# reazon-research/ReazonSpeech

Measured on NVIDIA H100. Metric: RTFx (audio-s/wall-s) FastConformer-RNNT 619M, higher is better.
Workload: dtype bf16

## Files before the change

reazonspeech_b200/csrc/attention_tc.cu:

```cuda
#include <cuda.h>

#include "common.cuh"
#include "kernels.h"

namespace rs {

namespace {

constexpr int TQ = 128;
constexpr int TDK = 128;
constexpr int KB = 64;
constexpr int kBlocks = 6;
constexpr int kSlab = TQ * 128;
constexpr int kAtcThreads = 32 * 9;
constexpr int kKvStages = 3;
constexpr uint32_t kKvStageBytes = 2 * KB * 128 + TDK * 128;
constexpr uint32_t kOffQ = 0;
constexpr uint32_t kOffKV = 2 * kSlab;
constexpr uint32_t kOffBD = kOffKV + kKvStages * kKvStageBytes;
constexpr int kBdPitch = 296;
constexpr int kNrelPadMax = 288;
constexpr uint32_t kOffBar = kOffBD + TQ * kBdPitch * 2;
constexpr uint32_t kAtcSmem = kOffBar + 1536 + 1024;
constexpr int kOutPitch = 136;
static_assert(2 * kNrelPadMax * 128 <= kKvStages * kKvStageBytes && kOutPitch <= kBdPitch && kAtcSmem <= 227 * 1024, "shared memory layout");

struct AtcDev {
  const __nv_bfloat16* qk;
  const __nv_bfloat16* vt;
  const float* bd_bias;
  const float* bias_u;
  __nv_bfloat16* out;
  const int32_t* enc_len;
  int T_max, H, w_left, w_right, n_global, n_rel_pad, ld_qk, ld_vt;
};

__device__ __forceinline__ float ex2f(float x) { float y; asm("ex2.approx.ftz.f32 %0, %1;" : "=f"(y) : "f"(x)); return y; }

__device__ __forceinline__ uint32_t sw128(int row, int chunk) {
  return static_cast<uint32_t>((row >> 3) * 1024 + (row & 7) * 128 + ((chunk ^ (row & 7)) << 4));
}

__global__ void __launch_bounds__(kAtcThreads, 1)
local_attention_tc_kernel(const __grid_constant__ CUtensorMap tm_q, const __grid_constant__ CUtensorMap tm_k,
                          const __grid_constant__ CUtensorMap tm_vt, const __grid_constant__ CUtensorMap tm_pos, const AtcDev p) {
  extern __shared__ uint8_t atc_raw[];
  const uint32_t base = (smem_u32(atc_raw) + 1023u) & ~1023u;
  uint8_t* gen = atc_raw + (base - smem_u32(atc_raw));
  const uint32_t bar_qk = base + kOffBar, bar_drained = bar_qk + 8;
  auto full_bar = [&](int s) { return bar_qk + 16u + 8u * s; };
  auto empty_bar = [&](int s) { return bar_qk + 40u + 8u * s; };
  __nv_bfloat16* s_k0 = reinterpret_cast<__nv_bfloat16*>(gen + kOffBar + 64);
  float* s_uk = reinterpret_cast<float*>(gen + kOffBar + 320);
  float* s_sg = reinterpret_cast<float*>(gen + kOffBar + 512);
  float* s_v0 = reinterpret_cast<float*>(gen + kOffBar + 1024);

  const int b = blockIdx.z, h = blockIdx.y, q0 = blockIdx.x * TQ;
  const int len = p.enc_len[b];
  const int d = p.H * TDK;
  const int warp = warp_id_uniform(), lane = lane_id();
  const size_t row0 = static_cast<size_t>(b) * p.T_max;
  __nv_bfloat16* obase = p.out + row0 * d + h * TDK;

  if (q0 >= len) {
    for (int id = threadIdx.x; id < TQ * 16; id += blockDim.x) {
      const int r = id >> 4, c = (id & 15) * 8;
      if (q0 + r < p.T_max) *reinterpret_cast<uint4*>(obase + static_cast<size_t>(q0 + r) * d + c) = make_uint4(0, 0, 0, 0);
    }
    return;
  }

  const int j_base = q0 - 128;
  const int q_hi = min(q0 + TQ, len) - 1;
  const int key_lo = max(0, q0 - p.w_left), key_hi = min(len - 1, q_hi + p.w_right);
  const int blk_lo = max((key_lo - j_base) >> 6, 0), blk_hi = min((key_hi - j_base) >> 6, kBlocks - 1);
  const uint32_t pos_slab = static_cast<uint32_t>(p.n_rel_pad) * 128u;

  if (threadIdx.x == 256) {
    tma_prefetch_desc(&tm_q);
    tma_prefetch_desc(&tm_k);
    tma_prefetch_desc(&tm_vt);
    tma_prefetch_desc(&tm_pos);
    mbar_init(bar_qk, 1); mbar_init(bar_drained, 8);
    for (int s = 0; s < kKvStages; ++s) { mbar_init(full_bar(s), 1); mbar_init(empty_bar(s), 8); }
    fence_barrier_init();
    mbar_arrive_expect_tx(bar_qk, static_cast<uint32_t>(2 * kSlab + 2 * pos_slab));
    for (int kb = 0; kb < 2; ++kb) {
      tma_load_2d(base + kOffQ + kb * kSlab, &tm_q, h * TDK + kb * 64, static_cast<int>(row0) + q0, bar_qk);
      for (int hh = 0; hh < 2; ++hh)
        tma_load_2d(base + kOffKV + kb * pos_slab + hh * (pos_slab / 2), &tm_pos, kb * 64, h * p.n_rel_pad + hh * (p.n_rel_pad / 2), bar_qk);
    }
  }
  __syncthreads();

  if (warp == 8) {
    if (lane == 0) {
      mbar_wait(bar_drained, 0);
      int s = 0; uint32_t phase = 0;
      for (int blk = blk_lo; blk <= blk_hi; ++blk) {
        mbar_wait(empty_bar(s), phase ^ 1u);
        mbar_arrive_expect_tx(full_bar(s), kKvStageBytes);
        const uint32_t st = base + kOffKV + s * kKvStageBytes;
        const int key0 = static_cast<int>(row0) + j_base + blk * KB;
        for (int kb = 0; kb < 2; ++kb) tma_load_2d(st + kb * (KB * 128), &tm_k, d + h * TDK + kb * 64, key0, full_bar(s));
        tma_load_2d(st + 2 * KB * 128, &tm_vt, key0, h * TDK, full_bar(s));
        if (++s == kKvStages) { s = 0; phase ^= 1u; }
      }
    }
    return;
  }

  const int wg = warp >> 2, g = lane >> 2, t = lane & 3;
  const int rbase = wg * 64 + (warp & 3) * 16;
  const int r0 = rbase + g, r1 = r0 + 8;
  const int i0 = q0 + r0, i1 = q0 + r1;
  const bool ok0 = i0 < len, ok1 = i1 < len;
  const float scale2 = rsqrtf(static_cast<float>(TDK)) * 1.4426950408889634f;
  __half* s_bd = reinterpret_cast<__half*>(gen + kOffBD);

  float sg0 = -INFINITY, sg1 = -INFINITY;
  if (p.n_global > 0) {
    const int tid = threadIdx.x;
    if (tid < 16) *reinterpret_cast<uint4*>(s_k0 + tid * 8) = __ldg(reinterpret_cast<const uint4*>(p.qk + row0 * p.ld_qk + d + h * TDK) + tid);
    if (tid >= 128) s_v0[tid - 128] = __bfloat162float(p.vt[static_cast<size_t>(h * TDK + (tid - 128)) * p.ld_vt + row0]);
    named_bar_sync(1, 256);
    if (warp == 0) {
      float uk = 0.f;
#pragma unroll
      for (int e = 0; e < 4; ++e) uk = fmaf(__ldg(p.bias_u + h * TDK + lane * 4 + e), __bfloat162float(s_k0[lane * 4 + e]), uk);
      uk = warp_sum(uk);
      if (lane == 0) *s_uk = uk;
    }
    mbar_wait(bar_qk, 0);
    {
      const int r = tid >> 1, hf = tid & 1;
      float acc0 = 0.f, acc1 = 0.f;
#pragma unroll
      for (int c = 0; c < 8; ++c) {
        const uint4 qv = *reinterpret_cast<const uint4*>(gen + kOffQ + hf * kSlab + sw128(r, c));
        const uint4 kv = *reinterpret_cast<const uint4*>(s_k0 + hf * 64 + c * 8);
        const uint32_t qw[4] = {qv.x, qv.y, qv.z, qv.w}, kw[4] = {kv.x, kv.y, kv.z, kv.w};
#pragma unroll
        for (int e = 0; e < 4; ++e) {
          const float2 q2 = unpack_bf16x2(qw[e]), k2 = unpack_bf16x2(kw[e]);
          acc0 = fmaf(q2.x, k2.x, acc0); acc1 = fmaf(q2.y, k2.y, acc1);
        }
      }
      float acc = acc0 + acc1;
      acc += __shfl_xor_sync(0xffffffffu, acc, 1);
      if (hf == 0) s_sg[r] = acc;
    }
    named_bar_sync(1, 256);
    sg0 = (s_sg[r0] - *s_uk) * scale2;
    sg1 = (s_sg[r1] - *s_uk) * scale2;
  } else {
    mbar_wait(bar_qk, 0);
  }

  const uint32_t q_addr = base + kOffQ + wg * (64 * 128);
#pragma unroll 1
  for (int ch = 0; ch < (p.n_rel_pad >> 5); ++ch) {
    float acc[16];
    wgmma_fence();
#pragma unroll
    for (int kb = 0; kb < 2; ++kb) {
      const uint64_t da = wgmma_desc_k_sw128(q_addr + kb * kSlab);
      const uint64_t db = wgmma_desc_k_sw128(base + kOffKV + kb * pos_slab + ch * 4096);
#pragma unroll
      for (int k = 0; k < 4; ++k) wgmma_bf16_ss_n32(acc, da + 2u * k, db + 2u * k, (kb | k) != 0 ? 1u : 0u);
    }
    wgmma_commit();
    wgmma_wait<0>();
#pragma unroll
    for (int j = 0; j < 4; ++j) {
      const int col = ch * 32 + 8 * j + 2 * t;
      const float2 bb = __ldg(reinterpret_cast<const float2*>(p.bd_bias + h * p.n_rel_pad + col));
      *reinterpret_cast<__half2*>(s_bd + r0 * kBdPitch + col) = __floats2half2_rn((acc[4 * j] + bb.x) * scale2, (acc[4 * j + 1] + bb.y) * scale2);
      *reinterpret_cast<__half2*>(s_bd + r1 * kBdPitch + col) = __floats2half2_rn((acc[4 * j + 2] + bb.x) * scale2, (acc[4 * j + 3] + bb.y) * scale2);
    }
  }
  __syncwarp();
  if (lane == 0) mbar_arrive(bar_drained);

  const int wrow_lo = q0 + wg * 64;
  const bool wg_valid = wrow_lo < len;
  const int wkey_lo = max(0, wrow_lo - p.w_left), wkey_hi = min(len - 1, min(wrow_lo + 64, len) - 1 + p.w_right);

  float o[64];
#pragma unroll
  for (int e = 0; e < 64; ++e) o[e] = 0.f;
  float m0 = -INFINITY, m1 = -INFINITY, l0 = 0.f, l1 = 0.f;
  const __half* bd0 = s_bd + r0 * kBdPitch + p.w_left - i0;
  const __half* bd1 = s_bd + r1 * kBdPitch + p.w_left - i1;
  int s = 0; uint32_t phase = 0;
#pragma unroll 1
  for (int blk = blk_lo; blk <= blk_hi; ++blk) {
    mbar_wait(full_bar(s), phase);
    const int jlo = j_base + blk * KB;
    if (wg_valid && jlo + KB - 1 >= wkey_lo && jlo <= wkey_hi) {
      const uint32_t st = base + kOffKV + s * kKvStageBytes;
      float sc[32];
      wgmma_fence();
#pragma unroll
      for (int kb = 0; kb < 2; ++kb) {
        const uint64_t da = wgmma_desc_k_sw128(q_addr + kb * kSlab);
        const uint64_t db = wgmma_desc_k_sw128(st + kb * (KB * 128));
#pragma unroll
        for (int k = 0; k < 4; ++k) wgmma_bf16_ss_n64(sc, da + 2u * k, db + 2u * k, (kb | k) != 0 ? 1u : 0u);
      }
      wgmma_commit();
      wgmma_wait<0>();
      float mx0 = -INFINITY, mx1 = -INFINITY;
#pragma unroll
      for (int j = 0; j < 8; ++j) {
#pragma unroll
        for (int q = 0; q < 2; ++q) {
          const int ja = jlo + 8 * j + 2 * t + q;
          const bool in = ja >= 0 && ja < len;
          const bool a0 = in && ok0 && ja - i0 >= -p.w_left && ja - i0 <= p.w_right;
          const bool a1 = in && ok1 && ja - i1 >= -p.w_left && ja - i1 <= p.w_right;
          const float t0 = a0 ? fmaf(sc[4 * j + q], scale2, __half2float(bd0[ja])) : -INFINITY;
          const float t1 = a1 ? fmaf(sc[4 * j + 2 + q], scale2, __half2float(bd1[ja])) : -INFINITY;
          sc[4 * j + q] = t0; sc[4 * j + 2 + q] = t1;
          mx0 = fmaxf(mx0, t0); mx1 = fmaxf(mx1, t1);
        }
      }
      mx0 = fmaxf(mx0, __shfl_xor_sync(0xffffffffu, mx0, 1)); mx0 = fmaxf(mx0, __shfl_xor_sync(0xffffffffu, mx0, 2));
      mx1 = fmaxf(mx1, __shfl_xor_sync(0xffffffffu, mx1, 1)); mx1 = fmaxf(mx1, __shfl_xor_sync(0xffffffffu, mx1, 2));
      const float n0 = fmaxf(m0, mx0), n1 = fmaxf(m1, mx1);
      const float c0 = m0 == -INFINITY ? 0.f : ex2f(m0 - n0), c1 = m1 == -INFINITY ? 0.f : ex2f(m1 - n1);
      const float ref0 = n0 == -INFINITY ? 0.f : n0, ref1 = n1 == -INFINITY ? 0.f : n1;
      m0 = n0; m1 = n1;
      l0 *= c0; l1 *= c1;
#pragma unroll
      for (int j = 0; j < 16; ++j) { o[4 * j] *= c0; o[4 * j + 1] *= c0; o[4 * j + 2] *= c1; o[4 * j + 3] *= c1; }
      uint32_t pa[4][4];
#pragma unroll
      for (int j = 0; j < 8; ++j) {
        const uint32_t w0 = pack_bf16x2(ex2f(sc[4 * j] - ref0), ex2f(sc[4 * j + 1] - ref0));
        const uint32_t w1 = pack_bf16x2(ex2f(sc[4 * j + 2] - ref1), ex2f(sc[4 * j + 3] - ref1));
        const float2 b0 = unpack_bf16x2(w0), b1 = unpack_bf16x2(w1);
        l0 += b0.x + b0.y; l1 += b1.x + b1.y;
        pa[j >> 1][(j & 1) * 2] = w0; pa[j >> 1][(j & 1) * 2 + 1] = w1;
      }
      wgmma_fence();
      const uint64_t dv = wgmma_desc_k_sw128(st + 2 * KB * 128);
#pragma unroll
      for (int kk = 0; kk < 4; ++kk) wgmma_bf16_rs_n128(o, pa[kk], dv + 2u * kk, 1u);
      wgmma_commit();
      wgmma_wait<0>();
    }
    __syncwarp();
    if (lane == 0) mbar_arrive(empty_bar(s));
    if (++s == kKvStages) { s = 0; phase ^= 1u; }
  }

  l0 += __shfl_xor_sync(0xffffffffu, l0, 1); l0 += __shfl_xor_sync(0xffffffffu, l0, 2);
  l1 += __shfl_xor_sync(0xffffffffu, l1, 1); l1 += __shfl_xor_sync(0xffffffffu, l1, 2);
  float pg0 = 0.f, pg1 = 0.f;
  if (p.n_global > 0) {
    const float f0 = fmaxf(m0, sg0), f1 = fmaxf(m1, sg1);
    const float c0 = m0 == -INFINITY ? 0.f : ex2f(m0 - f0), c1 = m1 == -INFINITY ? 0.f : ex2f(m1 - f1);
    pg0 = ok0 ? ex2f(sg0 - f0) : 0.f; pg1 = ok1 ? ex2f(sg1 - f1) : 0.f;
    l0 = l0 * c0 + pg0; l1 = l1 * c1 + pg1;
#pragma unroll
    for (int j = 0; j < 16; ++j) { o[4 * j] *= c0; o[4 * j + 1] *= c0; o[4 * j + 2] *= c1; o[4 * j + 3] *= c1; }
  }
  const float inv0 = (ok0 && l0 > 0.f) ? 1.0f / l0 : 0.f, inv1 = (ok1 && l1 > 0.f) ? 1.0f / l1 : 0.f;
  __syncwarp();
  __nv_bfloat16* stage = reinterpret_cast<__nv_bfloat16*>(s_bd + rbase * kBdPitch);
#pragma unroll
  for (int j = 0; j < 16; ++j) {
    const int col = 8 * j + 2 * t;
    const float v0a = p.n_global > 0 ? s_v0[col] : 0.f, v0b = p.n_global > 0 ? s_v0[col + 1] : 0.f;
    *reinterpret_cast<uint32_t*>(stage + g * kOutPitch + col) = pack_bf16x2((o[4 * j] + pg0 * v0a) * inv0, (o[4 * j + 1] + pg0 * v0b) * inv0);
    *reinterpret_cast<uint32_t*>(stage + (g + 8) * kOutPitch + col) = pack_bf16x2((o[4 * j + 2] + pg1 * v0a) * inv1, (o[4 * j + 3] + pg1 * v0b) * inv1);
  }
  __syncwarp();
#pragma unroll
  for (int it = 0; it < 8; ++it) {
    const int rr = it * 2 + (lane >> 4), cc = (lane & 15) * 8;
    const int row = q0 + rbase + rr;
    const uint4 a = *reinterpret_cast<const uint4*>(stage + rr * kOutPitch + cc);
    if (row < p.T_max) *reinterpret_cast<uint4*>(obase + static_cast<size_t>(row) * d + cc) = a;
  }
}

__global__ void __launch_bounds__(256)
global_row_attention_tc_kernel(const AtcDev p) {
  extern __shared__ __align__(16) float gs[];
  const int h = blockIdx.x, b = blockIdx.y;
  const int len = p.enc_len[b];
  if (len <= 0) return;
  const int d = p.H * TDK;
  const size_t row0 = static_cast<size_t>(b) * p.T_max;
  const __nv_bfloat16* qrow = p.qk + row0 * p.ld_qk + h * TDK;
  const __nv_bfloat16* kbase = qrow + d;
  const float scale = rsqrtf(static_cast<float>(TDK));
  const int tid = threadIdx.x, warp = tid >> 5, lane = tid & 31;
  const int t_pad = ((p.T_max > 1024 ? p.T_max : 1024) + 7) & ~7;
  float* red = gs + t_pad;
  float* sq = red + 8;
  if (tid < TDK) sq[tid] = (__bfloat162float(qrow[tid]) - p.bias_u[h * TDK + tid]) * scale;
  __syncthreads();
  float mx = -INFINITY;
  for (int j = tid; j < len; j += 256) {
    const uint4* kr = reinterpret_cast<const uint4*>(kbase + static_cast<size_t>(j) * p.ld_qk);
    uint4 kk[16];
#pragma unroll
    for (int i = 0; i < 16; ++i) kk[i] = __ldg(kr + i);
    float d0 = 0.f, d1 = 0.f, d2 = 0.f, d3 = 0.f;
#pragma unroll
    for (int i = 0; i < 16; ++i) {
      const float4 qa = *reinterpret_cast<const float4*>(sq + 8 * i), qb = *reinterpret_cast<const float4*>(sq + 8 * i + 4);
      d0 = fmaf(bf16_lo(kk[i].x), qa.x, d0); d1 = fmaf(bf16_hi(kk[i].x), qa.y, d1);
      d2 = fmaf(bf16_lo(kk[i].y), qa.z, d2); d3 = fmaf(bf16_hi(kk[i].y), qa.w, d3);
      d0 = fmaf(bf16_lo(kk[i].z), qb.x, d0); d1 = fmaf(bf16_hi(kk[i].z), qb.y, d1);
      d2 = fmaf(bf16_lo(kk[i].w), qb.z, d2); d3 = fmaf(bf16_hi(kk[i].w), qb.w, d3);
    }
    const float v = (d0 + d1) + (d2 + d3);
    gs[j] = v;
    mx = fmaxf(mx, v);
  }
  mx = warp_max(mx);
  if (lane == 0) red[warp] = mx;
  __syncthreads();
  mx = fmaxf(fmaxf(fmaxf(red[0], red[1]), fmaxf(red[2], red[3])), fmaxf(fmaxf(red[4], red[5]), fmaxf(red[6], red[7])));
  __syncthreads();
  float sum = 0.f;
  for (int j = tid; j < len; j += 256) { const float e = __expf(gs[j] - mx); gs[j] = e; sum += e; }
  sum = warp_sum(sum);
  if (lane == 0) red[warp] = sum;
  __syncthreads();
  const float inv = 1.0f / (((red[0] + red[1]) + (red[2] + red[3])) + ((red[4] + red[5]) + (red[6] + red[7])));
  __syncthreads();
  const __nv_bfloat16* vt = p.vt + static_cast<size_t>(h * TDK) * p.ld_vt + row0;
  const int len8 = ((row0 & 7) == 0) ? (len & ~7) : 0;
  const int dim = tid & 127, seg = tid >> 7;
  const int n8 = len8 >> 3;
  const int g_lo = seg == 0 ? 0 : (n8 + 1) / 2, g_hi = seg == 0 ? (n8 + 1) / 2 : n8;
  const __nv_bfloat16* vr = vt + static_cast<size_t>(dim) * p.ld_vt;
  float a0 = 0.f, a1 = 0.f, a2 = 0.f, a3 = 0.f;
  auto dot8 = [&](const uint4 raw, int j, float& acc) {
    const float4 p0 = *reinterpret_cast<const float4*>(gs + j), p1 = *reinterpret_cast<const float4*>(gs + j + 4);
    acc = fmaf(p0.x, bf16_lo(raw.x), acc); acc = fmaf(p0.y, bf16_hi(raw.x), acc);
    acc = fmaf(p0.z, bf16_lo(raw.y), acc); acc = fmaf(p0.w, bf16_hi(raw.y), acc);
    acc = fmaf(p1.x, bf16_lo(raw.z), acc); acc = fmaf(p1.y, bf16_hi(raw.z), acc);
    acc = fmaf(p1.z, bf16_lo(raw.w), acc); acc = fmaf(p1.w, bf16_hi(raw.w), acc);
  };
  int g = g_lo;
  for (; g + 4 <= g_hi; g += 4) {
    const uint4 r0 = __ldg(reinterpret_cast<const uint4*>(vr) + g), r1 = __ldg(reinterpret_cast<const uint4*>(vr) + g + 1);
    const uint4 r2 = __ldg(reinterpret_cast<const uint4*>(vr) + g + 2), r3 = __ldg(reinterpret_cast<const uint4*>(vr) + g + 3);
    dot8(r0, 8 * g, a0); dot8(r1, 8 * g + 8, a1); dot8(r2, 8 * g + 16, a2); dot8(r3, 8 * g + 24, a3);
  }
  for (; g < g_hi; ++g) dot8(__ldg(reinterpret_cast<const uint4*>(vr) + g), 8 * g, a0);
  if (seg == 1) for (int j = len8; j < len; ++j) a1 = fmaf(gs[j], __bfloat162float(vr[j]), a1);
  const float part = (a0 + a1) + (a2 + a3);
  __syncthreads();
  if (seg == 1) gs[dim] = part;
  __syncthreads();
  if (seg == 0) p.out[row0 * d + h * TDK + dim] = __float2bfloat16_rn((part + gs[dim]) * inv);
}

}

bool attention_tc_supported(const AttnArgs& a) {
  return a.dk == TDK && a.w_left >= 0 && a.w_right >= 0 && a.w_left <= 128 && a.w_right <= 128 && (a.w_left & 7) == 0 && a.n_global >= 0 &&
         a.n_global <= 1 && a.vt != nullptr && (a.T_max & 7) == 0 && a.n_rel_pad >= a.w_left + a.w_right + 1 && a.n_rel_pad % 32 == 0 &&
         a.n_rel_pad <= kNrelPadMax;
}

cudaError_t launch_attention_tc(const AttnArgs& a, cudaStream_t stream) {
  if (!attention_tc_supported(a) || a.pos == nullptr || a.bd_bias == nullptr || (a.ld_vt & 7)) return cudaErrorInvalidValue;
  const int d = a.H * TDK;
  const int64_t M = static_cast<int64_t>(a.B) * a.T_max;
  AtcDev p;
  p.qk = static_cast<const __nv_bfloat16*>(a.qkv); p.vt = static_cast<const __nv_bfloat16*>(a.vt);
  p.bd_bias = a.bd_bias; p.bias_u = a.bias_u; p.out = static_cast<__nv_bfloat16*>(a.out);
  p.enc_len = a.enc_len; p.T_max = a.T_max; p.H = a.H; p.w_left = a.w_left; p.w_right = a.w_right;
  p.n_global = a.n_global; p.n_rel_pad = a.n_rel_pad; p.ld_qk = 3 * d; p.ld_vt = a.ld_vt;
  CUtensorMap tm_q, tm_k, tm_vt, tm_pos;
  char err[256];
  if (!make_tmap_bf16(&tm_pos, a.pos, static_cast<uint64_t>(a.H) * a.n_rel_pad, TDK, TDK, static_cast<uint32_t>(a.n_rel_pad / 2), err)) return cudaErrorInvalidValue;
  if (!make_tmap_bf16(&tm_q, p.qk, static_cast<uint64_t>(M), static_cast<uint64_t>(2 * d), static_cast<uint64_t>(p.ld_qk), 128, err)) return cudaErrorInvalidValue;
  if (!make_tmap_bf16(&tm_k, p.qk, static_cast<uint64_t>(M), static_cast<uint64_t>(2 * d), static_cast<uint64_t>(p.ld_qk), KB, err)) return cudaErrorInvalidValue;
  if (!make_tmap_bf16(&tm_vt, p.vt, static_cast<uint64_t>(d), static_cast<uint64_t>(M), static_cast<uint64_t>(p.ld_vt), 128, err)) return cudaErrorInvalidValue;
  static DeviceOnce attr_once;
  if (attr_once.pending()) {
    cudaError_t e = cudaFuncSetAttribute(local_attention_tc_kernel, cudaFuncAttributeMaxDynamicSharedMemorySize, static_cast<int>(kAtcSmem));
    if (e != cudaSuccess) return e;
    e = cudaFuncSetAttribute(global_row_attention_tc_kernel, cudaFuncAttributeMaxDynamicSharedMemorySize, 200 * 1024);
    if (e != cudaSuccess) return e;
    attr_once.set();
  }
  const dim3 grid((a.T_max + TQ - 1) / TQ, a.H, a.B);
  local_attention_tc_kernel<<<grid, kAtcThreads, kAtcSmem, stream>>>(tm_q, tm_k, tm_vt, tm_pos, p);
  cudaError_t e = cudaGetLastError();
  if (e != cudaSuccess) return e;
  if (a.n_global > 0) {
    const size_t gsmem = (static_cast<size_t>(((a.T_max > 1024 ? a.T_max : 1024) + 7) & ~7) + 8 + TDK) * sizeof(float);
    if (gsmem > 200 * 1024) return cudaErrorInvalidValue;
    global_row_attention_tc_kernel<<<dim3(a.H, a.B), 256, gsmem, stream>>>(p);
    e = cudaGetLastError();
  }
  return e;
}

}
```

reazonspeech_b200/csrc/common.cuh:

```cuda
#pragma once
#include <cuda_bf16.h>
#include <cuda_fp16.h>
#include <cuda_runtime.h>
#include <stdint.h>

#include <atomic>

namespace rs {

struct DeviceOnce {
  std::atomic<unsigned long long> done{0};
  bool pending() const { int d = 0; cudaGetDevice(&d); return ((done.load(std::memory_order_acquire) >> (d & 63)) & 1ull) == 0; }
  void set() { int d = 0; cudaGetDevice(&d); done.fetch_or(1ull << (d & 63), std::memory_order_release); }
};

constexpr int kWarp = 32;

__device__ __forceinline__ uint32_t smem_u32(const void* p) {
  return static_cast<uint32_t>(__cvta_generic_to_shared(p));
}
__device__ __forceinline__ int lane_id() { return threadIdx.x & 31; }
__device__ __forceinline__ int warp_id_uniform() { return __shfl_sync(0xffffffffu, threadIdx.x >> 5, 0); }

__device__ __forceinline__ float warp_sum(float v) {
// ... 68 lines not shown
__device__ __forceinline__ void tma_load_2d(uint32_t smem_dst, const void* desc, int c0, int c1, uint32_t bar) {
  asm volatile(
      "cp.async.bulk.tensor.2d.shared::cluster.global.tile.mbarrier::complete_tx::bytes [%0], [%1, {%3, %4}], [%2];"
      ::"r"(smem_dst), "l"(desc), "r"(bar), "r"(c0), "r"(c1)
      : "memory");
}

__device__ __forceinline__ void tma_store_2d(const void* desc, uint32_t smem_src, int c0, int c1) {
  asm volatile("cp.async.bulk.tensor.2d.global.shared::cta.bulk_group [%0, {%2, %3}], [%1];"
               ::"l"(desc), "r"(smem_src), "r"(c0), "r"(c1) : "memory");
}
__device__ __forceinline__ void tma_reduce_add_2d(const void* desc, uint32_t smem_src, int c0, int c1) {
  asm volatile("cp.reduce.async.bulk.tensor.2d.global.shared::cta.add.tile.bulk_group [%0, {%2, %3}], [%1];"
               ::"l"(desc), "r"(smem_src), "r"(c0), "r"(c1) : "memory");
}
__device__ __forceinline__ void bulk_commit() { asm volatile("cp.async.bulk.commit_group;" ::: "memory"); }
template <int N>
__device__ __forceinline__ void bulk_wait_read() { asm volatile("cp.async.bulk.wait_group.read %0;" ::"n"(N) : "memory"); }
template <int N>
__device__ __forceinline__ void bulk_wait() { asm volatile("cp.async.bulk.wait_group %0;" ::"n"(N) : "memory"); }

__device__ __forceinline__ void cp_async16(void* smem, const void* gmem) {
  asm volatile("cp.async.cg.shared.global [%0], [%1], 16;" ::"r"(smem_u32(smem)), "l"(gmem) : "memory");
}
__device__ __forceinline__ void cp_async_wait_all() { asm volatile("cp.async.wait_all;" ::: "memory"); }

__device__ __forceinline__ void stmatrix_x4(uint32_t addr, uint32_t r0, uint32_t r1, uint32_t r2, uint32_t r3) {
  asm volatile("stmatrix.sync.aligned.m8n8.x4.shared.b16 [%0], {%1, %2, %3, %4};"
               ::"r"(addr), "r"(r0), "r"(r1), "r"(r2), "r"(r3) : "memory");
}
__device__ __forceinline__ void stmatrix_x4_trans(uint32_t addr, uint32_t r0, uint32_t r1, uint32_t r2, uint32_t r3) {
  asm volatile("stmatrix.sync.aligned.m8n8.x4.trans.shared.b16 [%0], {%1, %2, %3, %4};"
               ::"r"(addr), "r"(r0), "r"(r1), "r"(r2), "r"(r3) : "memory");
}

template <int N>
__device__ __forceinline__ void setmaxnreg_dec() { asm volatile("setmaxnreg.dec.sync.aligned.u32 %0;" ::"n"(N)); }
template <int N>
__device__ __forceinline__ void setmaxnreg_inc() { asm volatile("setmaxnreg.inc.sync.aligned.u32 %0;" ::"n"(N)); }

__device__ __forceinline__ void wgmma_fence() { asm volatile("wgmma.fence.sync.aligned;" ::: "memory"); }
__device__ __forceinline__ void wgmma_commit() { asm volatile("wgmma.commit_group.sync.aligned;" ::: "memory"); }
template <int N>
__device__ __forceinline__ void wgmma_wait() { asm volatile("wgmma.wait_group.sync.aligned %0;" ::"n"(N) : "memory"); }
__device__ __forceinline__ void named_bar_sync(int id, int threads) { asm volatile("bar.sync %0, %1;" ::"r"(id), "r"(threads) : "memory"); }

__device__ __forceinline__ uint64_t wgmma_desc_k_sw128(uint32_t smem_addr) {
  uint64_t d = 0;
  d |= static_cast<uint64_t>((smem_addr & 0x3ffffu) >> 4);
  d |= static_cast<uint64_t>(1) << 16;
  d |= static_cast<uint64_t>(1024 >> 4) << 32;
  d |= static_cast<uint64_t>(1) << 62;
  return d;
}

__device__ __forceinline__ void wgmma_bf16_ss_n32(float (&d)[16], uint64_t desc_a, uint64_t desc_b, uint32_t accumulate) {
  asm volatile(
      "{\n\t.reg .pred p;\n\t"
      "setp.ne.b32 p, %18, 0;\n\t"
      "wgmma.mma_async.sync.aligned.m64n32k16.f32.bf16.bf16 "
      "{%0, %1, %2, %3, %4, %5, %6, %7, %8, %9, %10, %11, %12, %13, %14, %15}, %16, %17, p, 1, 1, 0, 0;\n\t}"
      :
        "+f"(d[0]), "+f"(d[1]), "+f"(d[2]), "+f"(d[3]), "+f"(d[4]), "+f"(d[5]), "+f"(d[6]), "+f"(d[7]),
        "+f"(d[8]), "+f"(d[9]), "+f"(d[10]), "+f"(d[11]), "+f"(d[12]), "+f"(d[13]), "+f"(d[14]), "+f"(d[15])
      : "l"(desc_a), "l"(desc_b), "r"(accumulate));
}

__device__ __forceinline__ void wgmma_bf16_ss_n64(float (&d)[32], uint64_t desc_a, uint64_t desc_b, uint32_t accumulate) {
  asm volatile(
      "{\n\t.reg .pred p;\n\t"
      "setp.ne.b32 p, %34, 0;\n\t"
      "wgmma.mma_async.sync.aligned.m64n64k16.f32.bf16.bf16 "
      "{%0, %1, %2, %3, %4, %5, %6, %7, %8, %9, %10, %11, %12, %13, %14, %15, %16, %17, %18, %19, %20, %21, %22, %23, %24, %25, %26, %27, %28, %29, %30, %31}, %32, %33, p, 1, 1, 0, 0;\n\t}"
      :
        "+f"(d[0]), "+f"(d[1]), "+f"(d[2]), "+f"(d[3]), "+f"(d[4]), "+f"(d[5]), "+f"(d[6]), "+f"(d[7]),
        "+f"(d[8]), "+f"(d[9]), "+f"(d[10]), "+f"(d[11]), "+f"(d[12]), "+f"(d[13]), "+f"(d[14]), "+f"(d[15]),
        "+f"(d[16]), "+f"(d[17]), "+f"(d[18]), "+f"(d[19]), "+f"(d[20]), "+f"(d[21]), "+f"(d[22]), "+f"(d[23]),
        "+f"(d[24]), "+f"(d[25]), "+f"(d[26]), "+f"(d[27]), "+f"(d[28]), "+f"(d[29]), "+f"(d[30]), "+f"(d[31])
      : "l"(desc_a), "l"(desc_b), "r"(accumulate));
}

__device__ __forceinline__ void wgmma_bf16_ss_n128(float (&d)[64], uint64_t desc_a, uint64_t desc_b, uint32_t accumulate) {
  asm volatile(
      "{\n\t.reg .pred p;\n\t"
      "setp.ne.b32 p, %66, 0;\n\t"
      "wgmma.mma_async.sync.aligned.m64n128k16.f32.bf16.bf16 "
      "{%0, %1, %2, %3, %4, %5, %6, %7, %8, %9, %10, %11, %12, %13, %14, %15, %16, %17, %18, %19, %20, %21, %22, %23, %24, %25, %26, %27, %28, %29, %30, %31, %32, %33, %34, %35, %36, %37, %38, %39, %40, %41, %42, %43, %44, %45, %46, %47, %48, %49, %50, %51, %52, %53, %54, %55, %56, %57, %58, %59, %60, %61, %62, %63}, %64, %65, p, 1, 1, 0, 0;\n\t}"
      :
        "+f"(d[0]), "+f"(d[1]), "+f"(d[2]), "+f"(d[3]), "+f"(d[4]), "+f"(d[5]), "+f"(d[6]), "+f"(d[7]),
        "+f"(d[8]), "+f"(d[9]), "+f"(d[10]), "+f"(d[11]), "+f"(d[12]), "+f"(d[13]), "+f"(d[14]), "+f"(d[15]),
        "+f"(d[16]), "+f"(d[17]), "+f"(d[18]), "+f"(d[19]), "+f"(d[20]), "+f"(d[21]), "+f"(d[22]), "+f"(d[23]),
        "+f"(d[24]), "+f"(d[25]), "+f"(d[26]), "+f"(d[27]), "+f"(d[28]), "+f"(d[29]), "+f"(d[30]), "+f"(d[31]),
        "+f"(d[32]), "+f"(d[33]), "+f"(d[34]), "+f"(d[35]), "+f"(d[36]), "+f"(d[37]), "+f"(d[38]), "+f"(d[39]),
        "+f"(d[40]), "+f"(d[41]), "+f"(d[42]), "+f"(d[43]), "+f"(d[44]), "+f"(d[45]), "+f"(d[46]), "+f"(d[47]),
        "+f"(d[48]), "+f"(d[49]), "+f"(d[50]), "+f"(d[51]), "+f"(d[52]), "+f"(d[53]), "+f"(d[54]), "+f"(d[55]),
        "+f"(d[56]), "+f"(d[57]), "+f"(d[58]), "+f"(d[59]), "+f"(d[60]), "+f"(d[61]), "+f"(d[62]), "+f"(d[63])
      : "l"(desc_a), "l"(desc_b), "r"(accumulate));
}

__device__ __forceinline__ void wgmma_bf16_ss_n256(float (&d)[128], uint64_t desc_a, uint64_t desc_b, uint32_t accumulate) {
  asm volatile(
      "{\n\t.reg .pred p;\n\t"
      "setp.ne.b32 p, %130, 0;\n\t"
      "wgmma.mma_async.sync.aligned.m64n256k16.f32.bf16.bf16 "
      "{%0, %1, %2, %3, %4, %5, %6, %7, %8, %9, %10, %11, %12, %13, %14, %15, %16, %17, %18, %19, %20, %21, %22, %23, %24, %25, %26, %27, %28, %29, %30, %31, "
      "%32, %33, %34, %35, %36, %37, %38, %39, %40, %41, %42, %43, %44, %45, %46, %47, %48, %49, %50, %51, %52, %53, %54, %55, %56, %57, %58, %59, %60, %61, %62, %63, "
      "%64, %65, %66, %67, %68, %69, %70, %71, %72, %73, %74, %75, %76, %77, %78, %79, %80, %81, %82, %83, %84, %85, %86, %87, %88, %89, %90, %91, %92, %93, %94, %95, "
      "%96, %97, %98, %99, %100, %101, %102, %103, %104, %105, %106, %107, %108, %109, %110, %111, %112, %113, %114, %115, %116, %117, %118, %119, %120, %121, %122, %123, %124, %125, %126, %127}, "
      "%128, %129, p, 1, 1, 0, 0;\n\t}"
      :
        "+f"(d[0]), "+f"(d[1]), "+f"(d[2]), "+f"(d[3]), "+f"(d[4]), "+f"(d[5]), "+f"(d[6]), "+f"(d[7]),
        "+f"(d[8]), "+f"(d[9]), "+f"(d[10]), "+f"(d[11]), "+f"(d[12]), "+f"(d[13]), "+f"(d[14]), "+f"(d[15]),
        "+f"(d[16]), "+f"(d[17]), "+f"(d[18]), "+f"(d[19]), "+f"(d[20]), "+f"(d[21]), "+f"(d[22]), "+f"(d[23]),
        "+f"(d[24]), "+f"(d[25]), "+f"(d[26]), "+f"(d[27]), "+f"(d[28]), "+f"(d[29]), "+f"(d[30]), "+f"(d[31]),
        "+f"(d[32]), "+f"(d[33]), "+f"(d[34]), "+f"(d[35]), "+f"(d[36]), "+f"(d[37]), "+f"(d[38]), "+f"(d[39]),
        "+f"(d[40]), "+f"(d[41]), "+f"(d[42]), "+f"(d[43]), "+f"(d[44]), "+f"(d[45]), "+f"(d[46]), "+f"(d[47]),
        "+f"(d[48]), "+f"(d[49]), "+f"(d[50]), "+f"(d[51]), "+f"(d[52]), "+f"(d[53]), "+f"(d[54]), "+f"(d[55]),
        "+f"(d[56]), "+f"(d[57]), "+f"(d[58]), "+f"(d[59]), "+f"(d[60]), "+f"(d[61]), "+f"(d[62]), "+f"(d[63]),
// ... 52 lines not shown
```

Measured before the change: 22060.

## Stream pos/K/V through unified slot ring with warp-specialized, software-pipelined WGMMA attention

Replaces the fixed 3-stage K+V buffer and the up-front positional slab load with a 7-slot ring. One producer warp streams positional chunks, then K and V tiles separately through this ring, using setmaxnreg to shift registers from producers to consumers. Consumers double-buffer the accumulators so the next BD or QK WGMMA is issued while the current softmax and store run, and the BD GEMM moves to n64 tiles. Idle warpgroups and whole-block rows are zeroed per warp, and the global-attention kernel prefetches keys and V rows before the reductions. This adds substantial barrier bookkeeping (skipped-block acquire/release, parity per element) and register pressure, with a risk of deadlock or spills.

```diff
diff --git a/reazonspeech_b200/csrc/attention_tc.cu b/reazonspeech_b200/csrc/attention_tc.cu
--- a/reazonspeech_b200/csrc/attention_tc.cu
+++ b/reazonspeech_b200/csrc/attention_tc.cu
@@ -12,18 +12,19 @@
 constexpr int KB = 64;
 constexpr int kBlocks = 6;
 constexpr int kSlab = TQ * 128;
-constexpr int kAtcThreads = 32 * 9;
-constexpr int kKvStages = 3;
-constexpr uint32_t kKvStageBytes = 2 * KB * 128 + TDK * 128;
+constexpr int kAtcThreads = 32 * 12;
+constexpr int kProducerRegs = 24, kConsumerRegs = 240;
+constexpr int kSlots = 7;
+constexpr uint32_t kSlotBytes = 2 * KB * 128;
 constexpr uint32_t kOffQ = 0;
 constexpr uint32_t kOffKV = 2 * kSlab;
-constexpr uint32_t kOffBD = kOffKV + kKvStages * kKvStageBytes;
+constexpr uint32_t kOffBD = kOffKV + kSlots * kSlotBytes;
 constexpr int kBdPitch = 296;
 constexpr int kNrelPadMax = 288;
 constexpr uint32_t kOffBar = kOffBD + TQ * kBdPitch * 2;
 constexpr uint32_t kAtcSmem = kOffBar + 1536 + 1024;
 constexpr int kOutPitch = 136;
-static_assert(2 * kNrelPadMax * 128 <= kKvStages * kKvStageBytes && kOutPitch <= kBdPitch && kAtcSmem <= 227 * 1024, "shared memory layout");
+static_assert(TDK * KB * 2 == kSlotBytes && kNrelPadMax <= kBdPitch && kOutPitch <= kBdPitch && kAtcSmem <= 227 * 1024, "shared memory layout");
 
 struct AtcDev {
   const __nv_bfloat16* qk;
@@ -41,17 +42,23 @@
   return static_cast<uint32_t>((row >> 3) * 1024 + (row & 7) * 128 + ((chunk ^ (row & 7)) << 4));
 }
 
+template <int N>
+__device__ __forceinline__ void fence_regs(float (&r)[N]) {
+#pragma unroll
+  for (int i = 0; i < N; ++i) asm volatile("" : "+f"(r[i])::"memory");
+}
+
 __global__ void __launch_bounds__(kAtcThreads, 1)
 local_attention_tc_kernel(const __grid_constant__ CUtensorMap tm_q, const __grid_constant__ CUtensorMap tm_k,
                           const __grid_constant__ CUtensorMap tm_vt, const __grid_constant__ CUtensorMap tm_pos, const AtcDev p) {
   extern __shared__ uint8_t atc_raw[];
   const uint32_t base = (smem_u32(atc_raw) + 1023u) & ~1023u;
   uint8_t* gen = atc_raw + (base - smem_u32(atc_raw));
-  const uint32_t bar_qk = base + kOffBar, bar_drained = bar_qk + 8;
-  auto full_bar = [&](int s) { return bar_qk + 16u + 8u * s; };
-  auto empty_bar = [&](int s) { return bar_qk + 40u + 8u * s; };
-  __nv_bfloat16* s_k0 = reinterpret_cast<__nv_bfloat16*>(gen + kOffBar + 64);
-  float* s_uk = reinterpret_cast<float*>(gen + kOffBar + 320);
+  const uint32_t bar_qk = base + kOffBar;
+  auto full_bar = [&](int s) { return bar_qk + 8u + 8u * s; };
+  auto empty_bar = [&](int s) { return bar_qk + 8u + 8u * kSlots + 8u * s; };
+  __nv_bfloat16* s_k0 = reinterpret_cast<__nv_bfloat16*>(gen + kOffBar + 128);
+  float* s_uk = reinterpret_cast<float*>(gen + kOffBar + 384);
   float* s_sg = reinterpret_cast<float*>(gen + kOffBar + 512);
   float* s_v0 = reinterpret_cast<float*>(gen + kOffBar + 1024);
 
@@ -62,11 +69,15 @@
   const size_t row0 = static_cast<size_t>(b) * p.T_max;
   __nv_bfloat16* obase = p.out + row0 * d + h * TDK;
 
+  auto zero_rows16 = [&](int r) {
+#pragma unroll
+    for (int it = 0; it < 8; ++it) {
+      const int row = q0 + r + it * 2 + (lane >> 4), cc = (lane & 15) * 8;
+      if (row < p.T_max) *reinterpret_cast<uint4*>(obase + static_cast<size_t>(row) * d + cc) = make_uint4(0, 0, 0, 0);
+    }
+  };
   if (q0 >= len) {
-    for (int id = threadIdx.x; id < TQ * 16; id += blockDim.x) {
-      const int r = id >> 4, c = (id & 15) * 8;
-      if (q0 + r < p.T_max) *reinterpret_cast<uint4*>(obase + static_cast<size_t>(q0 + r) * d + c) = make_uint4(0, 0, 0, 0);
-    }
+    if (warp < 8) zero_rows16(warp * 16);
     return;
   }
 
@@ -74,42 +85,53 @@
   const int q_hi = min(q0 + TQ, len) - 1;
   const int key_lo = max(0, q0 - p.w_left), key_hi = min(len - 1, q_hi + p.w_right);
   const int blk_lo = max((key_lo - j_base) >> 6, 0), blk_hi = min((key_hi - j_base) >> 6, kBlocks - 1);
-  const uint32_t pos_slab = static_cast<uint32_t>(p.n_rel_pad) * 128u;
+  const int n_pos = (p.n_rel_pad + KB - 1) / KB;
+  const int n_stream = n_pos + 2 * (blk_hi - blk_lo + 1);
+  const int n_wg = q0 + 64 < len ? 2 : 1;
+  auto slot_parity = [](int e) { return static_cast<uint32_t>((e / kSlots) & 1); };
+  auto slot_addr = [&](int e) { return base + kOffKV + (e % kSlots) * kSlotBytes; };
 
   if (threadIdx.x == 256) {
     tma_prefetch_desc(&tm_q);
     tma_prefetch_desc(&tm_k);
     tma_prefetch_desc(&tm_vt);
     tma_prefetch_desc(&tm_pos);
-    mbar_init(bar_qk, 1); mbar_init(bar_drained, 8);
-    for (int s = 0; s < kKvStages; ++s) { mbar_init(full_bar(s), 1); mbar_init(empty_bar(s), 8); }
+    mbar_init(bar_qk, 1);
+    for (int s = 0; s < kSlots; ++s) { mbar_init(full_bar(s), 1); mbar_init(empty_bar(s), 4 * n_wg); }
     fence_barrier_init();
-    mbar_arrive_expect_tx(bar_qk, static_cast<uint32_t>(2 * kSlab + 2 * pos_slab));
-    for (int kb = 0; kb < 2; ++kb) {
-      tma_load_2d(base + kOffQ + kb * kSlab, &tm_q, h * TDK + kb * 64, static_cast<int>(row0) + q0, bar_qk);
-      for (int hh = 0; hh < 2; ++hh)
-        tma_load_2d(base + kOffKV + kb * pos_slab + hh * (pos_slab / 2), &tm_pos, kb * 64, h * p.n_rel_pad + hh * (p.n_rel_pad / 2), bar_qk);
-    }
-  }
-  __syncthreads();
-
-  if (warp == 8) {
-    if (lane == 0) {
-      mbar_wait(bar_drained, 0);
-      int s = 0; uint32_t phase = 0;
-      for (int blk = blk_lo; blk <= blk_hi; ++blk) {
-        mbar_wait(empty_bar(s), phase ^ 1u);
-        mbar_arrive_expect_tx(full_bar(s), kKvStageBytes);
-        const uint32_t st = base + kOffKV + s * kKvStageBytes;
-        const int key0 = static_cast<int>(row0) + j_base + blk * KB;
-        for (int kb = 0; kb < 2; ++kb) tma_load_2d(st + kb * (KB * 128), &tm_k, d + h * TDK + kb * 64, key0, full_bar(s));
-        tma_load_2d(st + 2 * KB * 128, &tm_vt, key0, h * TDK, full_bar(s));
-        if (++s == kKvStages) { s = 0; phase ^= 1u; }
+    mbar_arrive_expect_tx(bar_qk, static_cast<uint32_t>(2 * kSlab));
+    for (int kb = 0; kb < 2; ++kb) tma_load_2d(base + kOffQ + kb * kSlab, &tm_q, h * TDK + kb * 64, static_cast<int>(row0) + q0, bar_qk);
+  }
+  __syncthreads();
+
+  if (warp >= 8) {
+    setmaxnreg_dec<kProducerRegs>();
+    if (warp == 8 && lane == 0) {
+      for (int e = 0; e < n_stream; ++e) {
+        const int s = e % kSlots;
+        mbar_wait(empty_bar(s), slot_parity(e) ^ 1u);
+        const uint32_t st = slot_addr(e);
+        if (e < n_pos) {
+          const int boxes = min(KB, p.n_rel_pad - e * KB) / 32;
+          mbar_arrive_expect_tx(full_bar(s), static_cast<uint32_t>(boxes * 2 * 32 * 128));
+          for (int kb = 0; kb < 2; ++kb)
+            for (int hh = 0; hh < boxes; ++hh)
+              tma_load_2d(st + kb * (KB * 128) + hh * (32 * 128), &tm_pos, kb * 64, h * p.n_rel_pad + e * KB + hh * 32, full_bar(s));
+        } else {
+          mbar_arrive_expect_tx(full_bar(s), kSlotBytes);
+          const int key0 = static_cast<int>(row0) + j_base + (blk_lo + (e - n_pos) / 2) * KB;
+          if (((e - n_pos) & 1) == 0) {
+            for (int kb = 0; kb < 2; ++kb) tma_load_2d(st + kb * (KB * 128), &tm_k, d + h * TDK + kb * 64, key0, full_bar(s));
+          } else {
+            tma_load_2d(st, &tm_vt, key0, h * TDK, full_bar(s));
+          }
+        }
       }
     }
     return;
   }
 
+  setmaxnreg_inc<kConsumerRegs>();
   const int wg = warp >> 2, g = lane >> 2, t = lane & 3;
   const int rbase = wg * 64 + (warp & 3) * 16;
   const int r0 = rbase + g, r1 = r0 + 8;
@@ -118,7 +140,6 @@
   const float scale2 = rsqrtf(static_cast<float>(TDK)) * 1.4426950408889634f;
   __half* s_bd = reinterpret_cast<__half*>(gen + kOffBD);
 
-  float sg0 = -INFINITY, sg1 = -INFINITY;
   if (p.n_global > 0) {
     const int tid = threadIdx.x;
     if (tid < 16) *reinterpret_cast<uint4*>(s_k0 + tid * 8) = __ldg(reinterpret_cast<const uint4*>(p.qk + row0 * p.ld_qk + d + h * TDK) + tid);
@@ -151,40 +172,75 @@
       if (hf == 0) s_sg[r] = acc;
     }
     named_bar_sync(1, 256);
-    sg0 = (s_sg[r0] - *s_uk) * scale2;
-    sg1 = (s_sg[r1] - *s_uk) * scale2;
   } else {
     mbar_wait(bar_qk, 0);
   }
-
+  if (wg >= n_wg) {
+    zero_rows16(rbase);
+    return;
+  }
+
+  auto acquire = [&](int e) { mbar_wait(full_bar(e % kSlots), slot_parity(e)); };
+  auto release = [&](int e) {
+    __syncwarp();
+    if (lane == 0) mbar_arrive(empty_bar(e % kSlots));
+  };
   const uint32_t q_addr = base + kOffQ + wg * (64 * 128);
+  {
+    float ba[32], bb[32];
+#pragma unroll
+    for (int e = 0; e < 32; ++e) { ba[e] = 0.f; bb[e] = 0.f; }
+    fence_regs(ba); fence_regs(bb);
+    auto bd_issue = [&](float (&acc)[32], int c) {
+      acquire(c);
+      const uint32_t st = slot_addr(c);
+      wgmma_fence();
+#pragma unroll
+      for (int kb = 0; kb < 2; ++kb) {
+        const uint64_t da = wgmma_desc_k_sw128(q_addr + kb * kSlab), db = wgmma_desc_k_sw128(st + kb * (KB * 128));
+#pragma unroll
+        for (int k = 0; k < 4; ++k) wgmma_bf16_ss_n64(acc, da + 2u * k, db + 2u * k, (kb | k) != 0 ? 1u : 0u);
+      }
+      wgmma_commit();
+    };
+    auto bd_step = [&](float (&acc)[32], float (&next)[32], int c) {
+      float2 bias[8];
+#pragma unroll
+      for (int j = 0; j < 8; ++j)
+        bias[j] = c * KB + 8 * j < p.n_rel_pad ? __ldg(reinterpret_cast<const float2*>(p.bd_bias + h * p.n_rel_pad + c * KB + 8 * j + 2 * t))
+                                               : make_float2(0.f, 0.f);
+      wgmma_wait<0>();
+      release(c);
+      if (c + 1 < n_pos) bd_issue(next, c + 1);
+#pragma unroll
+      for (int j = 0; j < 8; ++j) {
+        const int col = c * KB + 8 * j + 2 * t;
+        if (c * KB + 8 * j < p.n_rel_pad) {
+          *reinterpret_cast<__half2*>(s_bd + r0 * kBdPitch + col) = __floats2half2_rn((acc[4 * j] + bias[j].x) * scale2, (acc[4 * j + 1] + bias[j].y) * scale2);
+          *reinterpret_cast<__half2*>(s_bd + r1 * kBdPitch + col) = __floats2half2_rn((acc[4 * j + 2] + bias[j].x) * scale2, (acc[4 * j + 3] + bias[j].y) * scale2);
+        }
+      }
+    };
+    bd_issue(ba, 0);
 #pragma unroll 1
-  for (int ch = 0; ch < (p.n_rel_pad >> 5); ++ch) {
-    float acc[16];
-    wgmma_fence();
-#pragma unroll
-    for (int kb = 0; kb < 2; ++kb) {
-      const uint64_t da = wgmma_desc_k_sw128(q_addr + kb * kSlab);
-      const uint64_t db = wgmma_desc_k_sw128(base + kOffKV + kb * pos_slab + ch * 4096);
-#pragma unroll
-      for (int k = 0; k < 4; ++k) wgmma_bf16_ss_n32(acc, da + 2u * k, db + 2u * k, (kb | k) != 0 ? 1u : 0u);
-    }
-    wgmma_commit();
-    wgmma_wait<0>();
-#pragma unroll
-    for (int j = 0; j < 4; ++j) {
-      const int col = ch * 32 + 8 * j + 2 * t;
-      const float2 bb = __ldg(reinterpret_cast<const float2*>(p.bd_bias + h * p.n_rel_pad + col));
-      *reinterpret_cast<__half2*>(s_bd + r0 * kBdPitch + col) = __floats2half2_rn((acc[4 * j] + bb.x) * scale2, (acc[4 * j + 1] + bb.y) * scale2);
-      *reinterpret_cast<__half2*>(s_bd + r1 * kBdPitch + col) = __floats2half2_rn((acc[4 * j + 2] + bb.x) * scale2, (acc[4 * j + 3] + bb.y) * scale2);
+    for (int c = 0; c < n_pos; c += 2) {
+      bd_step(ba, bb, c);
+      if (c + 1 < n_pos) bd_step(bb, ba, c + 1);
     }
   }
   __syncwarp();
-  if (lane == 0) mbar_arrive(bar_drained);
 
   const int wrow_lo = q0 + wg * 64;
-  const bool wg_valid = wrow_lo < len;
   const int wkey_lo = max(0, wrow_lo - p.w_left), wkey_hi = min(len - 1, min(wrow_lo + 64, len) - 1 + p.w_right);
+  int a_lo = blk_hi + 1, a_hi = blk_hi;
+  for (int blk = blk_lo; blk <= blk_hi; ++blk) {
+    const int jlo = j_base + blk * KB;
+    if (jlo + KB - 1 >= wkey_lo && jlo <= wkey_hi) { a_lo = min(a_lo, blk); a_hi = blk; }
+  }
+  const bool rows_full = wrow_lo + 64 <= len;
+  auto k_elem = [&](int blk) { return n_pos + 2 * (blk - blk_lo); };
+  for (int blk = blk_lo; blk < a_lo; ++blk)
+    for (int e = k_elem(blk); e <= k_elem(blk) + 1; ++e) { acquire(e); release(e); }
 
   float o[64];
 #pragma unroll
@@ -192,25 +248,41 @@
   float m0 = -INFINITY, m1 = -INFINITY, l0 = 0.f, l1 = 0.f;
   const __half* bd0 = s_bd + r0 * kBdPitch + p.w_left - i0;
   const __half* bd1 = s_bd + r1 * kBdPitch + p.w_left - i1;
-  int s = 0; uint32_t phase = 0;
-#pragma unroll 1
-  for (int blk = blk_lo; blk <= blk_hi; ++blk) {
-    mbar_wait(full_bar(s), phase);
+  uint32_t pa[4][4];
+  float sa[32], sb[32];
+#pragma unroll
+  for (int e = 0; e < 32; ++e) { sa[e] = 0.f; sb[e] = 0.f; }
+  fence_regs(sa); fence_regs(sb); fence_regs(o);
+  auto s_issue = [&](float (&sc)[32], int blk) {
+    acquire(k_elem(blk));
+    const uint32_t st = slot_addr(k_elem(blk));
+    wgmma_fence();
+#pragma unroll
+    for (int kb = 0; kb < 2; ++kb) {
+      const uint64_t da = wgmma_desc_k_sw128(q_addr + kb * kSlab);
+      const uint64_t db = wgmma_desc_k_sw128(st + kb * (KB * 128));
+#pragma unroll
+      for (int k = 0; k < 4; ++k) wgmma_bf16_ss_n64(sc, da + 2u * k, db + 2u * k, (kb | k) != 0 ? 1u : 0u);
+    }
+    wgmma_commit();
+  };
+  auto step = [&](float (&sc)[32], float (&sn)[32], int blk) {
     const int jlo = j_base + blk * KB;
-    if (wg_valid && jlo + KB - 1 >= wkey_lo && jlo <= wkey_hi) {
-      const uint32_t st = base + kOffKV + s * kKvStageBytes;
-      float sc[32];
-      wgmma_fence();
-#pragma unroll
-      for (int kb = 0; kb < 2; ++kb) {
-        const uint64_t da = wgmma_desc_k_sw128(q_addr + kb * kSlab);
-        const uint64_t db = wgmma_desc_k_sw128(st + kb * (KB * 128));
-#pragma unroll
-        for (int k = 0; k < 4; ++k) wgmma_bf16_ss_n64(sc, da + 2u * k, db + 2u * k, (kb | k) != 0 ? 1u : 0u);
+    float mx0 = -INFINITY, mx1 = -INFINITY;
+    const bool interior = rows_full && jlo >= 0 && jlo + KB <= len && jlo - (wrow_lo + 63) >= -p.w_left && jlo + KB - 1 - wrow_lo <= p.w_right;
+    if (interior) {
+#pragma unroll
+      for (int j = 0; j < 8; ++j) {
+#pragma unroll
+        for (int q = 0; q < 2; ++q) {
+          const int ja = jlo + 8 * j + 2 * t + q;
+          const float t0 = fmaf(sc[4 * j + q], scale2, __half2float(bd0[ja]));
+          const float t1 = fmaf(sc[4 * j + 2 + q], scale2, __half2float(bd1[ja]));
+          sc[4 * j + q] = t0; sc[4 * j + 2 + q] = t1;
+          mx0 = fmaxf(mx0, t0); mx1 = fmaxf(mx1, t1);
+        }
       }
-      wgmma_commit();
-      wgmma_wait<0>();
-      float mx0 = -INFINITY, mx1 = -INFINITY;
+    } else {
 #pragma unroll
       for (int j = 0; j < 8; ++j) {
 #pragma unroll
@@ -225,40 +297,53 @@
           mx0 = fmaxf(mx0, t0); mx1 = fmaxf(mx1, t1);
         }
       }
-      mx0 = fmaxf(mx0, __shfl_xor_sync(0xffffffffu, mx0, 1)); mx0 = fmaxf(mx0, __shfl_xor_sync(0xffffffffu, mx0, 2));
-      mx1 = fmaxf(mx1, __shfl_xor_sync(0xffffffffu, mx1, 1)); mx1 = fmaxf(mx1, __shfl_xor_sync(0xffffffffu, mx1, 2));
-      const float n0 = fmaxf(m0, mx0), n1 = fmaxf(m1, mx1);
-      const float c0 = m0 == -INFINITY ? 0.f : ex2f(m0 - n0), c1 = m1 == -INFINITY ? 0.f : ex2f(m1 - n1);
-      const float ref0 = n0 == -INFINITY ? 0.f : n0, ref1 = n1 == -INFINITY ? 0.f : n1;
-      m0 = n0; m1 = n1;
-      l0 *= c0; l1 *= c1;
-#pragma unroll
-      for (int j = 0; j < 16; ++j) { o[4 * j] *= c0; o[4 * j + 1] *= c0; o[4 * j + 2] *= c1; o[4 * j + 3] *= c1; }
-      uint32_t pa[4][4];
-#pragma unroll
-      for (int j = 0; j < 8; ++j) {
-        const uint32_t w0 = pack_bf16x2(ex2f(sc[4 * j] - ref0), ex2f(sc[4 * j + 1] - ref0));
-        const uint32_t w1 = pack_bf16x2(ex2f(sc[4 * j + 2] - ref1), ex2f(sc[4 * j + 3] - ref1));
-        const float2 b0 = unpack_bf16x2(w0), b1 = unpack_bf16x2(w1);
-        l0 += b0.x + b0.y; l1 += b1.x + b1.y;
-        pa[j >> 1][(j & 1) * 2] = w0; pa[j >> 1][(j & 1) * 2 + 1] = w1;
-      }
-      wgmma_fence();
-      const uint64_t dv = wgmma_desc_k_sw128(st + 2 * KB * 128);
-#pragma unroll
-      for (int kk = 0; kk < 4; ++kk) wgmma_bf16_rs_n128(o, pa[kk], dv + 2u * kk, 1u);
-      wgmma_commit();
-      wgmma_wait<0>();
-    }
-    __syncwarp();
-    if (lane == 0) mbar_arrive(empty_bar(s));
-    if (++s == kKvStages) { s = 0; phase ^= 1u; }
-  }
+    }
+    mx0 = fmaxf(mx0, __shfl_xor_sync(0xffffffffu, mx0, 1)); mx0 = fmaxf(mx0, __shfl_xor_sync(0xffffffffu, mx0, 2));
+    mx1 = fmaxf(mx1, __shfl_xor_sync(0xffffffffu, mx1, 1)); mx1 = fmaxf(mx1, __shfl_xor_sync(0xffffffffu, mx1, 2));
+    const float n0 = fmaxf(m0, mx0), n1 = fmaxf(m1, mx1);
+    const float c0 = m0 == -INFINITY ? 0.f : ex2f(m0 - n0), c1 = m1 == -INFINITY ? 0.f : ex2f(m1 - n1);
+    const float ref0 = n0 == -INFINITY ? 0.f : n0, ref1 = n1 == -INFINITY ? 0.f : n1;
+    m0 = n0; m1 = n1;
+    l0 *= c0; l1 *= c1;
+#pragma unroll
+    for (int j = 0; j < 16; ++j) { o[4 * j] *= c0; o[4 * j + 1] *= c0; o[4 * j + 2] *= c1; o[4 * j + 3] *= c1; }
+#pragma unroll
+    for (int j = 0; j < 8; ++j) {
+      const uint32_t w0 = pack_bf16x2(ex2f(sc[4 * j] - ref0), ex2f(sc[4 * j + 1] - ref0));
+      const uint32_t w1 = pack_bf16x2(ex2f(sc[4 * j + 2] - ref1), ex2f(sc[4 * j + 3] - ref1));
+      const float2 b0 = unpack_bf16x2(w0), b1 = unpack_bf16x2(w1);
+      l0 += b0.x + b0.y; l1 += b1.x + b1.y;
+      pa[j >> 1][(j & 1) * 2] = w0; pa[j >> 1][(j & 1) * 2 + 1] = w1;
+    }
+    if (blk < a_hi) s_issue(sn, blk + 1);
+    acquire(k_elem(blk) + 1);
+    wgmma_fence();
+    const uint64_t dv = wgmma_desc_k_sw128(slot_addr(k_elem(blk) + 1));
+#pragma unroll
+    for (int kk = 0; kk < 4; ++kk) wgmma_bf16_rs_n128(o, pa[kk], dv + 2u * kk, 1u);
+    wgmma_commit();
+    wgmma_wait<0>();
+    release(k_elem(blk) + 1);
+    if (blk < a_hi) release(k_elem(blk + 1));
+  };
+  if (a_lo <= a_hi) {
+    s_issue(sa, a_lo);
+    wgmma_wait<0>();
+    release(k_elem(a_lo));
+#pragma unroll 1
+    for (int blk = a_lo; blk <= a_hi; blk += 2) {
+      step(sa, sb, blk);
+      if (blk + 1 <= a_hi) step(sb, sa, blk + 1);
+    }
+  }
+  for (int blk = a_hi + 1; blk <= blk_hi; ++blk)
+    for (int e = k_elem(blk); e <= k_elem(blk) + 1; ++e) { acquire(e); release(e); }
 
   l0 += __shfl_xor_sync(0xffffffffu, l0, 1); l0 += __shfl_xor_sync(0xffffffffu, l0, 2);
   l1 += __shfl_xor_sync(0xffffffffu, l1, 1); l1 += __shfl_xor_sync(0xffffffffu, l1, 2);
   float pg0 = 0.f, pg1 = 0.f;
   if (p.n_global > 0) {
+    const float sg0 = (s_sg[r0] - *s_uk) * scale2, sg1 = (s_sg[r1] - *s_uk) * scale2;
     const float f0 = fmaxf(m0, sg0), f1 = fmaxf(m1, sg1);
     const float c0 = m0 == -INFINITY ? 0.f : ex2f(m0 - f0), c1 = m1 == -INFINITY ? 0.f : ex2f(m1 - f1);
     pg0 = ok0 ? ex2f(sg0 - f0) : 0.f; pg1 = ok1 ? ex2f(sg1 - f1) : 0.f;
@@ -301,14 +386,18 @@
   const int t_pad = ((p.T_max > 1024 ? p.T_max : 1024) + 7) & ~7;
   float* red = gs + t_pad;
   float* sq = red + 8;
+  uint4 kk[16];
+  auto load_key = [&](int j) {
+    const uint4* kr = reinterpret_cast<const uint4*>(kbase + static_cast<size_t>(j) * p.ld_qk);
+#pragma unroll
+    for (int i = 0; i < 16; ++i) kk[i] = __ldg(kr + i);
+  };
+  if (tid < len) load_key(tid);
   if (tid < TDK) sq[tid] = (__bfloat162float(qrow[tid]) - p.bias_u[h * TDK + tid]) * scale;
   __syncthreads();
   float mx = -INFINITY;
   for (int j = tid; j < len; j += 256) {
-    const uint4* kr = reinterpret_cast<const uint4*>(kbase + static_cast<size_t>(j) * p.ld_qk);
-    uint4 kk[16];
-#pragma unroll
-    for (int i = 0; i < 16; ++i) kk[i] = __ldg(kr + i);
+    if (j != tid) load_key(j);
     float d0 = 0.f, d1 = 0.f, d2 = 0.f, d3 = 0.f;
 #pragma unroll
     for (int i = 0; i < 16; ++i) {
@@ -322,24 +411,31 @@
     gs[j] = v;
     mx = fmaxf(mx, v);
   }
-  mx = warp_max(mx);
-  if (lane == 0) red[warp] = mx;
-  __syncthreads();
-  mx = fmaxf(fmaxf(fmaxf(red[0], red[1]), fmaxf(red[2], red[3])), fmaxf(fmaxf(red[4], red[5]), fmaxf(red[6], red[7])));
-  __syncthreads();
-  float sum = 0.f;
-  for (int j = tid; j < len; j += 256) { const float e = __expf(gs[j] - mx); gs[j] = e; sum += e; }
-  sum = warp_sum(sum);
-  if (lane == 0) red[warp] = sum;
-  __syncthreads();
-  const float inv = 1.0f / (((red[0] + red[1]) + (red[2] + red[3])) + ((red[4] + red[5]) + (red[6] + red[7])));
-  __syncthreads();
   const __nv_bfloat16* vt = p.vt + static_cast<size_t>(h * TDK) * p.ld_vt + row0;
   const int len8 = ((row0 & 7) == 0) ? (len & ~7) : 0;
   const int dim = tid & 127, seg = tid >> 7;
   const int n8 = len8 >> 3;
   const int g_lo = seg == 0 ? 0 : (n8 + 1) / 2, g_hi = seg == 0 ? (n8 + 1) / 2 : n8;
   const __nv_bfloat16* vr = vt + static_cast<size_t>(dim) * p.ld_vt;
+  constexpr int kPre = 12;
+  const bool pre = g_hi - g_lo >= kPre;
+  uint4 vpre[kPre];
+  if (pre) {
+#pragma unroll
+    for (int i = 0; i < kPre; ++i) vpre[i] = __ldg(reinterpret_cast<const uint4*>(vr) + g_lo + i);
+  }
+  mx = warp_max(mx);
+  if (lane == 0) red[warp] = mx;
+  __syncthreads();
+  mx = fmaxf(fmaxf(fmaxf(red[0], red[1]), fmaxf(red[2], red[3])), fmaxf(fmaxf(red[4], red[5]), fmaxf(red[6], red[7])));
+  __syncthreads();
+  float sum = 0.f;
+  for (int j = tid; j < len; j += 256) { const float e = __expf(gs[j] - mx); gs[j] = e; sum += e; }
+  sum = warp_sum(sum);
+  if (lane == 0) red[warp] = sum;
+  __syncthreads();
+  const float inv = 1.0f / (((red[0] + red[1]) + (red[2] + red[3])) + ((red[4] + red[5]) + (red[6] + red[7])));
+  __syncthreads();
   float a0 = 0.f, a1 = 0.f, a2 = 0.f, a3 = 0.f;
   auto dot8 = [&](const uint4 raw, int j, float& acc) {
     const float4 p0 = *reinterpret_cast<const float4*>(gs + j), p1 = *reinterpret_cast<const float4*>(gs + j + 4);
@@ -349,6 +445,14 @@
     acc = fmaf(p1.z, bf16_lo(raw.w), acc); acc = fmaf(p1.w, bf16_hi(raw.w), acc);
   };
   int g = g_lo;
+  if (pre) {
+#pragma unroll
+    for (int i = 0; i < kPre; i += 4) {
+      dot8(vpre[i], 8 * (g + i), a0); dot8(vpre[i + 1], 8 * (g + i) + 8, a1);
+      dot8(vpre[i + 2], 8 * (g + i) + 16, a2); dot8(vpre[i + 3], 8 * (g + i) + 24, a3);
+    }
+    g += kPre;
+  }
   for (; g + 4 <= g_hi; g += 4) {
     const uint4 r0 = __ldg(reinterpret_cast<const uint4*>(vr) + g), r1 = __ldg(reinterpret_cast<const uint4*>(vr) + g + 1);
     const uint4 r2 = __ldg(reinterpret_cast<const uint4*>(vr) + g + 2), r3 = __ldg(reinterpret_cast<const uint4*>(vr) + g + 3);
@@ -382,7 +486,7 @@
   p.n_global = a.n_global; p.n_rel_pad = a.n_rel_pad; p.ld_qk = 3 * d; p.ld_vt = a.ld_vt;
   CUtensorMap tm_q, tm_k, tm_vt, tm_pos;
   char err[256];
-  if (!make_tmap_bf16(&tm_pos, a.pos, static_cast<uint64_t>(a.H) * a.n_rel_pad, TDK, TDK, static_cast<uint32_t>(a.n_rel_pad / 2), err)) return cudaErrorInvalidValue;
+  if (!make_tmap_bf16(&tm_pos, a.pos, static_cast<uint64_t>(a.H) * a.n_rel_pad, TDK, TDK, 32, err)) return cudaErrorInvalidValue;
   if (!make_tmap_bf16(&tm_q, p.qk, static_cast<uint64_t>(M), static_cast<uint64_t>(2 * d), static_cast<uint64_t>(p.ld_qk), 128, err)) return cudaErrorInvalidValue;
   if (!make_tmap_bf16(&tm_k, p.qk, static_cast<uint64_t>(M), static_cast<uint64_t>(2 * d), static_cast<uint64_t>(p.ld_qk), KB, err)) return cudaErrorInvalidValue;
   if (!make_tmap_bf16(&tm_vt, p.vt, static_cast<uint64_t>(d), static_cast<uint64_t>(M), static_cast<uint64_t>(p.ld_vt), 128, err)) return cudaErrorInvalidValue;
diff --git a/reazonspeech_b200/csrc/common.cuh b/reazonspeech_b200/csrc/common.cuh
--- a/reazonspeech_b200/csrc/common.cuh
+++ b/reazonspeech_b200/csrc/common.cuh
@@ -144,18 +144,6 @@
   d |= static_cast<uint64_t>(1024 >> 4) << 32;
   d |= static_cast<uint64_t>(1) << 62;
   return d;
-}
-
-__device__ __forceinline__ void wgmma_bf16_ss_n32(float (&d)[16], uint64_t desc_a, uint64_t desc_b, uint32_t accumulate) {
-  asm volatile(
-      "{\n\t.reg .pred p;\n\t"
-      "setp.ne.b32 p, %18, 0;\n\t"
-      "wgmma.mma_async.sync.aligned.m64n32k16.f32.bf16.bf16 "
-      "{%0, %1, %2, %3, %4, %5, %6, %7, %8, %9, %10, %11, %12, %13, %14, %15}, %16, %17, p, 1, 1, 0, 0;\n\t}"
-      :
-        "+f"(d[0]), "+f"(d[1]), "+f"(d[2]), "+f"(d[3]), "+f"(d[4]), "+f"(d[5]), "+f"(d[6]), "+f"(d[7]),
-        "+f"(d[8]), "+f"(d[9]), "+f"(d[10]), "+f"(d[11]), "+f"(d[12]), "+f"(d[13]), "+f"(d[14]), "+f"(d[15])
-      : "l"(desc_a), "l"(desc_b), "r"(accumulate));
 }
 
 __device__ __forceinline__ void wgmma_bf16_ss_n64(float (&d)[32], uint64_t desc_a, uint64_t desc_b, uint32_t accumulate) {
```

Result: no change. 22200, median of 6 (+0.6%).
